# crockwell/far

Hardware: AMD Instinct MI355X
Metric: image-pairs/sec (match+solve+regress) at 640x480 (higher is better)
Workload: dtype f32

## Files before the change

### far_amd/csrc/mlp_fused_f16s.hip

```cpp
#include "common.h"

namespace {

typedef _Float16 f16x8 __attribute__((ext_vector_type(8)));
typedef __attribute__((address_space(3))) void* lptr_t;

constexpr int DM = 128;
constexpr int KIN = 2 * DM;
constexpr int HID = 2 * DM;
constexpr int NS1 = KIN / 16;
constexpr int HT = HID / 32;
constexpr int CT = DM / 32;
constexpr int SLAB = 16384;
constexpr int NSLAB = NS1 + HT;
constexpr int RING = 3;
constexpr int WAVES = 4;
constexpr int PIECES = 16 / WAVES;
constexpr float ACT_SCALE = 16.0f;

__device__ __forceinline__ void glds16(const void* gsrc, unsigned lds_dst_uniform) {
    unsigned keep;
    asm volatile("s_mov_b32 %0, m0\n\ts_mov_b32 m0, %2\n\ts_nop 0\n\tglobal_load_lds_dwordx4 %1, off\n\ts_mov_b32 m0, %0"
                 : "=&s"(keep) : "v"(gsrc), "s"(lds_dst_uniform) : "memory");
}

__device__ __forceinline__ void split8(const float4& u, const float4& v, float scale, f16x8& hi, f16x8& lo) {
    const float x[8] = {u.x, u.y, u.z, u.w, v.x, v.y, v.z, v.w};
#pragma unroll
    for (int i = 0; i < 8; i += 2) {
        f16x2 h, l;
        split2(f32x2{x[i], x[i + 1]} * f32x2{scale, scale}, h, l);
        hi[i] = h.x; hi[i + 1] = h.y;
        lo[i] = l.x; lo[i + 1] = l.y;
    }
}

#define FAR_DPP_F(v, ctrl) __builtin_bit_cast(float, __builtin_amdgcn_update_dpp(0, __builtin_bit_cast(int, v), ctrl, 0xF, 0xF, true))
__device__ __forceinline__ float sum32(float v) {
    v += FAR_DPP_F(v, 0xB1);
    v += FAR_DPP_F(v, 0x4E);
    v += FAR_DPP_F(v, 0x141);
    v += FAR_DPP_F(v, 0x140);
    return v + shfl_xor_f(v, 16);
}


template <bool SPLIT, bool LGKM = true>
__global__ __launch_bounds__(256, 2) void k_mlp128(const float* __restrict__ x, const float* __restrict__ msg,
                                                   const unsigned char* __restrict__ wimg, long R, float hscale, float oscale,
                                                   const float* __restrict__ gamma, const float* __restrict__ beta, float eps,
                                                   float* __restrict__ out, int* __restrict__ overflow) {
    __shared__ __attribute__((aligned(16))) unsigned char ring[RING * SLAB];
    __shared__ __attribute__((aligned(16))) unsigned char xs[WAVES * 4096];
    const int tid = threadIdx.x, lane = tid & 63, l31 = lane & 31, h = lane >> 5;
    const int wave = __builtin_amdgcn_readfirstlane(tid >> 6);
    const long row0 = (long)blockIdx.x * (32 * WAVES) + 32 * wave;
    const unsigned ring_base = (unsigned)__builtin_amdgcn_readfirstlane((int)(unsigned)(size_t)(lptr_t)ring);
    const unsigned xs_base = (unsigned)__builtin_amdgcn_readfirstlane((int)(unsigned)(size_t)(lptr_t)(xs + wave * 4096));
    const unsigned char* wsrc = wimg + (size_t)lane * 16;
    auto request_w = [&](int s) {
        const unsigned dst = ring_base + (unsigned)((s % RING) * SLAB);
#pragma unroll
        for (int i = 0; i < PIECES; ++i)
            glds16(wsrc + (size_t)s * SLAB + (wave + WAVES * i) * 1024, dst + (wave + WAVES * i) * 1024);
    };
    const int rr = lane >> 3, q = lane & 7;
    auto request_x = [&](int c) {
        const float* base = (c < 4 ? x : msg) + 32 * (c & 3);
        const unsigned dst = xs_base;
#pragma unroll
        for (int j = 0; j < 4; ++j) {
            const int r = 8 * j + rr;
            long gr = row0 + r;
            gr = gr < R ? gr : R - 1;
            glds16(base + gr * DM + 4 * (q ^ ((r ^ (r >> 3)) & 7)), dst + j * 1024);
        }
    };
    request_x(0);
    request_w(0);
    request_w(1);
    f16x8 xh[2], xl[2];
    f32x16 acc1[HT];
#pragma unroll
    for (int t = 0; t < HT; ++t)
#pragma unroll
        for (int r = 0; r < 16; ++r) acc1[t][r] = 0.f;
    const unsigned char* xrd = xs + wave * 4096 + (l31 >> 3) * 1024 + (l31 & 7) * 128;
    const int sw = (l31 ^ (l31 >> 3)) & 7;

#pragma unroll
    for (int s = 0; s < NS1; ++s) {
        asm volatile("s_waitcnt vmcnt(0)" ::: "memory");
        ring_barrier<LGKM>();
        if ((s & 1) == 0) {
            float4 raw[4];
#pragma unroll
            for (int i = 0; i < 4; ++i) raw[i] = *reinterpret_cast<const float4*>(xrd + (((4 * h + i) ^ sw) * 16));
            asm volatile("s_waitcnt lgkmcnt(0)" ::: "memory");
            if ((s >> 1) + 1 < KIN / 32) request_x((s >> 1) + 1);
            split8(raw[0], raw[1], ACT_SCALE, xh[0], xl[0]);
            split8(raw[2], raw[3], ACT_SCALE, xh[1], xl[1]);
        }
        request_w(s + 2);
        const unsigned char* slab = ring + (s % RING) * SLAB + lane * 16;
        const f16x8 bh = xh[s & 1], bl = xl[s & 1];
        f16x8 ah[3], al[3];
#pragma unroll
        for (int t = 0; t < 2; ++t) {
            ah[t] = *reinterpret_cast<const f16x8*>(slab + t * 2048);
            al[t] = *reinterpret_cast<const f16x8*>(slab + t * 2048 + 1024);
        }
#pragma unroll
        for (int t = 0; t < HT; ++t) {
            if (t + 2 < HT) {
                ah[(t + 2) % 3] = *reinterpret_cast<const f16x8*>(slab + (t + 2) * 2048);
                al[(t + 2) % 3] = *reinterpret_cast<const f16x8*>(slab + (t + 2) * 2048 + 1024);
            }
            acc1[t] = __builtin_amdgcn_mfma_f32_32x32x16_f16(ah[t % 3], bh, acc1[t], 0, 0, 0);
            if (SPLIT) {
                acc1[t] = __builtin_amdgcn_mfma_f32_32x32x16_f16(ah[t % 3], bl, acc1[t], 0, 0, 0);
                acc1[t] = __builtin_amdgcn_mfma_f32_32x32x16_f16(al[t % 3], bh, acc1[t], 0, 0, 0);
            }
            __builtin_amdgcn_sched_group_barrier(0x100, SPLIT ? 2 : 1, 0);
            __builtin_amdgcn_sched_group_barrier(0x008, SPLIT ? 3 : 1, 0);
        }
    }

    f32x16 acc2[CT];
    float hid_chk = 0.f;
#pragma unroll
    for (int ct = 0; ct < CT; ++ct)
#pragma unroll
        for (int r = 0; r < 16; ++r) acc2[ct][r] = 0.f;
#pragma unroll
    for (int t = 0; t < HT; ++t) {
        const int s = NS1 + t;
        asm volatile("s_waitcnt vmcnt(0)" ::: "memory");
        ring_barrier<LGKM>();
        if (s + 2 < NSLAB) request_w(s + 2);
        const unsigned char* slab = ring + (s % RING) * SLAB + lane * 16;
        f16x8 ha[2], hl[2];
#pragma unroll
        for (int u = 0; u < 2; ++u)
#pragma unroll
            for (int e = 0; e < 8; e += 2) {
                hid_chk += acc1[t][8 * u + e] + acc1[t][8 * u + e + 1];
                const f32x2 hv = __builtin_elementwise_max(f32x2{acc1[t][8 * u + e], acc1[t][8 * u + e + 1]} * f32x2{hscale, hscale}, f32x2{0.f, 0.f});
                f16x2 h2, l2;
                split2(hv, h2, l2);
                ha[u][e] = h2.x; ha[u][e + 1] = h2.y;
                hl[u][e] = l2.x; hl[u][e + 1] = l2.y;
            }
        f16x8 bh[3], bl[3];
#pragma unroll
        for (int i = 0; i < 2; ++i) {
            bh[i] = *reinterpret_cast<const f16x8*>(slab + (i * 2) * 1024);
            bl[i] = *reinterpret_cast<const f16x8*>(slab + (i * 2 + 1) * 1024);
        }
#pragma unroll
        for (int i = 0; i < 2 * CT; ++i) {
            if (i + 2 < 2 * CT) {
                bh[(i + 2) % 3] = *reinterpret_cast<const f16x8*>(slab + ((i + 2) * 2) * 1024);
                bl[(i + 2) % 3] = *reinterpret_cast<const f16x8*>(slab + ((i + 2) * 2 + 1) * 1024);
            }
            const int u = i / CT, ct = i % CT;
            acc2[ct] = __builtin_amdgcn_mfma_f32_32x32x16_f16(ha[u], bh[i % 3], acc2[ct], 0, 0, 0);
            if (SPLIT) {
                acc2[ct] = __builtin_amdgcn_mfma_f32_32x32x16_f16(ha[u], bl[i % 3], acc2[ct], 0, 0, 0);
                acc2[ct] = __builtin_amdgcn_mfma_f32_32x32x16_f16(hl[u], bh[i % 3], acc2[ct], 0, 0, 0);
            }
            __builtin_amdgcn_sched_group_barrier(0x100, SPLIT ? 2 : 1, 0);
            __builtin_amdgcn_sched_group_barrier(0x008, SPLIT ? 3 : 1, 0);
        }
    }

    if (overflow) {
        float chk = hid_chk;
#pragma unroll
        for (int ct = 0; ct < CT; ++ct)
#pragma unroll
            for (int r = 0; r < 16; ++r) chk += acc2[ct][r];
        if (__any(!(fabsf(chk) <= FLT_MAX)) && (threadIdx.x & 63) == 0) atomicOr(overflow, 1);
    }
    const float inv_c = 1.0f / (float)DM;
    float g[CT], b[CT];
#pragma unroll
    for (int ct = 0; ct < CT; ++ct) { g[ct] = gamma[32 * ct + l31]; b[ct] = beta[32 * ct + l31]; }
#pragma unroll
    for (int r = 0; r < 16; ++r) {
        float v[CT];
        float sum = 0.f;
#pragma unroll
        for (int ct = 0; ct < CT; ++ct) { v[ct] = acc2[ct][r] * oscale; sum += v[ct]; }
        const float mean = sum32(sum) * inv_c;
        float sq = 0.f;
#pragma unroll
        for (int ct = 0; ct < CT; ++ct) { v[ct] -= mean; sq += v[ct] * v[ct]; }
        const float rstd = 1.0f / sqrtf(sum32(sq) * inv_c + eps);
        const long orow = row0 + mfma32_row(r, h);
        if (orow < R) {
#pragma unroll
            for (int ct = 0; ct < CT; ++ct) {
                const long o = orow * DM + 32 * ct + l31;
                out[o] = x[o] + (v[ct] * rstd * g[ct] + b[ct]);
            }
        }
    }
}

template <bool SPLIT>
int mlp_fused_launch(const float* x, const float* msg, const void* packed, long R, int d_model, float hscale, float oscale,
                     const float* gamma, const float* beta, float eps, float* out, int* overflow, hipStream_t stream) {
    far_clear_errors();
    if (R == 0) return FAR_OK;
    if (!x || !msg || !packed || !gamma || !beta || !out || R < 0 || d_model != DM || out == x || out == msg) return FAR_EINVAL;
    const long nb = (R + 32 * WAVES - 1) / (32 * WAVES);
    if (nb > 0x7fffffffL) return FAR_EINVAL;
#ifdef FAR_RING_EXP
    if (far_get_tuning(11) & 4) {
        hipLaunchKernelGGL((k_mlp128<SPLIT, false>), dim3((unsigned)nb), dim3(64 * WAVES), 0, stream, x, msg, (const unsigned char*)packed, R,
                           hscale, oscale, gamma, beta, eps, out, overflow);
        return far_check_launch();
    }
#endif
    hipLaunchKernelGGL(k_mlp128<SPLIT>, dim3((unsigned)nb), dim3(64 * WAVES), 0, stream, x, msg, (const unsigned char*)packed, R, hscale,
                       oscale, gamma, beta, eps, out, overflow);
    return far_check_launch();
}

}

extern "C" {

size_t far_mlp_fused_packed_bytes(int d_model) { return d_model == DM ? (size_t)NSLAB * SLAB : 0; }

int far_mlp_fused_f16s(const float* x, const float* msg, const void* packed, long R, int d_model, float hscale, float oscale,
                       const float* gamma, const float* beta, float eps, float* out, int* overflow, hipStream_t stream) {
    return mlp_fused_launch<true>(x, msg, packed, R, d_model, hscale, oscale, gamma, beta, eps, out, overflow, stream);
}

int far_mlp_fused_f16(const float* x, const float* msg, const void* packed, long R, int d_model, float hscale, float oscale,
                      const float* gamma, const float* beta, float eps, float* out, int* overflow, hipStream_t stream) {
    return mlp_fused_launch<false>(x, msg, packed, R, d_model, hscale, oscale, gamma, beta, eps, out, overflow, stream);
}

}
```

### far_amd/flags.py

```python
import os
from collections import namedtuple

Switch = namedtuple('Switch', 'env module attr off_value neutral scope doc')
SWITCHES = [
    Switch('FAR_NO_WINO', 'far_amd.ops', 'USE_WINO', False, 'parity', 'inference',
           'stride-1 3x3 convolutions on K9 (direct implicit GEMM) instead of K17 (Winograd F(2x2,3x3)); same operator, other summation'),
    Switch('FAR_NO_PAD', 'far_amd.loftr.backbone', 'PAD_CHANNELS', False, 'bitwise', 'inference',
           'the 196-channel backbone maps stored with 196 channels instead of 208 (zero weights for the extra ones: exact zeros)'),
    Switch('FAR_NO_PREFETCH', 'far_amd.loftr.model:LoFTR', 'head_prefetch', False, 'bitwise', 'inference',
           "the head's feature stage computed inside forward_rt_prediction instead of enqueued behind K1"),
    Switch('FAR_NO_SIDE_STREAM', 'far_amd.loftr.model:LoFTR', 'head_side_stream', False, 'bitwise', 'inference',
           "the head's feature stage on the step's own stream behind K1 (rounds 2-5) instead of on a second stream next to K1 and the fine level"),
    Switch('FAR_FPN_STREAM', 'far_amd.loftr.model:LoFTR', 'fpn_side_stream', True, 'bitwise', 'inference',
           "OPT-IN (1 switches it ON; default off): the FPN's fine branch on a side stream next to the coarse transformer and K1 (-0.6 ms per 32 "
           "pairs; off by default because the roofline launch -- K17 208 -> 208 @ 240x320 -- then shares the GPU and its in-step duration "
           "in a kernel trace is no longer its own)"),
    Switch('FAR_NO_GATHER_FUSE', 'far_amd.loftr.stages:FinePreprocess', 'fused_gather', False, 'bitwise', 'inference',
           'FinePreprocess.merge_feat on a materialised window tensor (K3 gather + K9) instead of K9 reading through the match indices'),
    Switch('FAR_NO_KV', 'far_amd.loftr.transformer:LoFTREncoderLayer', 'fused_kv', False, 'parity', 'inference',
           "k, v projections + K5's first half as separate launches instead of K9's k|v epilogue (the K'^T V sum changes order)"),
    Switch('FAR_NO_QAPPLY', 'far_amd.loftr.transformer:LoFTREncoderLayer', 'fused_apply', False, 'parity', 'inference',
           "q projection + K5's second half as separate launches instead of K9's attention-apply epilogue (q no longer stays in split operands)"),
    Switch('FAR_NO_STACK', 'far_amd.loftr.transformer:LocalFeatureTransformer', 'stack_self', False, 'bitwise', 'inference',
           "the two 'self' calls of an encoder layer on the two images separately instead of one call on both"),
    Switch('FAR_NO_BN', 'far_amd.ops', 'USE_HIP_BATCHNORM_TRAIN', False, 'parity', 'training',
           'training-mode BatchNorm on nn.BatchNorm2d + torch activations instead of K19 (tests/test_train_kernels_gpu.py holds K19 to the module)'),
]

ENV_ONLY = {
    'FAR_HIP_LIB': ('load', 'path of another build of libfar_hip.so (tools/ab_build.py: same-box A/B against a git revision); skips the build-id check'),
    'FAR_TUNING': ('load', 'comma-separated key=value pairs handed to far_set_tuning at load time, e.g. FAR_TUNING="10=1,8=1" (keys below)'),
    'FAR_SKIP_ASM_CHECK': ('build', "1: far_amd/build.py does not scan the generated code (K9's asm pixel loads; the LDS-DMA ring rule of every kernel with global_load_lds; the half-register writes of the asm fp16 split) after recompiling"),
    'FAR_EXTRA_HIPCC_FLAGS': ('build', 'extra hipcc flags of an experiment build (-DFAR_WINO_EXP=..., tools/wino_exp.sh); part of the build id'),
    'FAR_COMMIT': ('tools', 'commit stamp tools/collect_profiles.sh / tools/step_floors.py write into the profile files'),
    'FAR_C3_PY_NODE': ('bench', "bench.py --workload c3: the encoder layer's autograd node driven from Python instead of far_enc_layer_fwd / _bwd"),
    'FAR_C3_NO_OVERLAP': ('bench', 'bench.py --workload c3: the layer node without side streams'),
    'FAR_C3_PER_OP': ('bench', 'bench.py --workload c3: one autograd node per operator instead of per layer'),
    'FAR_TORCH_ADAMW': ('bench', 'bench.py --workload c3: torch.optim.AdamW instead of K20'),
    'FAR_CUDNN_BENCHMARK': ('bench', 'bench.py: torch.backends.cudnn.benchmark for the vendor comparison legs'),
}

Tuning = namedtuple('Tuning', 'key default values neutral doc')
TUNING = [
    Tuning(0, 3, (0, 1, 2, 4, 7), 'bitwise', 'bit mask of exact-f32 kernels that stagger wave-slot priorities: 1 k_stats, 2 k_match, 4 k_emm_pv'),
    Tuning(1, 0, (1,), 'parity', 'K1 exact-f32 variant: the other tile shape (another summation order of the row statistics)'),
    Tuning(2, 0, (1,), 'bitwise', 'conf_matrix writer variant A (store pattern)'),
    Tuning(3, 0, (1,), 'bitwise', 'conf_matrix writer variant B (store pattern)'),
    Tuning(4, 0, (1,), 'bitwise', 'K9 without the seven-tile mode / K5 windows on the generic path'),
    Tuning(5, 0, (1, 2, 4), 'bitwise', 'K5 apply: tiles per unit'),
    Tuning(6, 0, (64, 256), 'parity', "K5: tokens per K'^T V chunk (another partial-sum grouping)"),
    Tuning(7, 0, (1,), 'bitwise', 'K9 Linear launches always on full-height tiles'),
    Tuning(8, 0, (1,), 'bitwise', 'K17 splits its operands with the five-instruction split2 instead of v_fma_mix (same values)'),
    Tuning(9, 0, (1,), 'bitwise', 'K17 runs a short last channel block on the full body'),
    Tuning(10, 0, (1,), 'bitwise', "K1's match pass without the tile prescreen"),
    Tuning(11, 0, (1, 2), 'bitwise', "K14's pipeline: 0 = 4 waves / 3 slots / counted waits, two workgroups per CU; 1 = 8 waves / 4 slots / counted, one per CU (round 5's form); 2 = 4 waves / 3 slots / vmcnt(0) per phase (fallback without a wait table)"),
    Tuning(12, 0, (1,), 'parity', "K10's inference form on the exact-f32 matrix instruction instead of split fp16"),
    Tuning(15, 0, (1,), 'bitwise', 'K17: 1 = the multiplying wave group does NOT raise its issue priority (the round-4 kernel)'),
    Tuning(13, 0, (1,), 'bitwise', "K9's FPN-merge epilogue in its generic form everywhere"),
]


def off(env):
    if env not in {s.env for s in SWITCHES}:
        raise KeyError(f'{env} is not a registered far_amd switch (far_amd/flags.py)')
    return os.environ.get(env, '0') not in ('', '0')


def value(env, default=None):
    if env not in ENV_ONLY:
        raise KeyError(f'{env} is not a registered far_amd environment variable (far_amd/flags.py)')
    return os.environ.get(env, default)


def known():
    return {s.env for s in SWITCHES} | set(ENV_ONLY)


def unknown_in_environment():
    skip = ('FAR_WINO_', 'FAR_K9_')
    return sorted(k for k in os.environ if k.startswith('FAR_') and k not in known() and not k.startswith(skip))


def target(sw):
    import importlib
    mod, _, cls = sw.module.partition(':')
    obj = importlib.import_module(mod)
    return (getattr(obj, cls) if cls else obj), sw.attr
```

Before: 371.7.

## Double-buffer MLP input chunks, count vmcnt waits, batch residual loads

The fused MLP kernel gets a second per-wave LDS input slot so each activation chunk is requested two phases ahead. The blanket vmcnt(0) waits are replaced by counted waits taken from a compile-time table, so a phase waits only for the loads it actually reads. The epilogue also fetches all residual x values in one batch before the layer norm, and uses an unguarded store path for full tiles. LDS moves to dynamic shared memory, which raises per-block usage by one more input buffer per wave and could reduce occupancy. A tuning knob keeps the older variants available.

```diff
diff --git a/far_amd/csrc/mlp_fused_f16s.hip b/far_amd/csrc/mlp_fused_f16s.hip
--- a/far_amd/csrc/mlp_fused_f16s.hip
+++ b/far_amd/csrc/mlp_fused_f16s.hip
@@ -1,4 +1,5 @@
 #include "common.h"
+#include <type_traits>
 
 namespace {
 
@@ -16,6 +17,7 @@
 constexpr int RING = 3;
 constexpr int WAVES = 4;
 constexpr int PIECES = 16 / WAVES;
+constexpr int XBUF = 4096;
 constexpr float ACT_SCALE = 16.0f;
 
 __device__ __forceinline__ void glds16(const void* gsrc, unsigned lds_dst_uniform) {
@@ -44,19 +46,59 @@
     return v + shfl_xor_f(v, 16);
 }
 
-
-template <bool SPLIT, bool LGKM = true>
+constexpr int chunk_read_in_phase(int s) { return (s < NS1 && (s & 1) == 0) ? s / 2 : -1; }
+constexpr int vm_allow(int p, int xb) {
+    int kind[64] = {}, id[64] = {}, n[64] = {}, cnt = 0;
+    for (int c0 = 0; c0 < xb; ++c0) { kind[cnt] = 0; id[cnt] = c0; n[cnt++] = 4; }
+    for (int s0 = 0; s0 < RING - 1; ++s0) { kind[cnt] = 1; id[cnt] = s0; n[cnt++] = PIECES; }
+    for (int s = 0; s < p; ++s) {
+        const int c = chunk_read_in_phase(s);
+        if (c >= 0 && c + xb < KIN / 32) { kind[cnt] = 0; id[cnt] = c + xb; n[cnt++] = 4; }
+        if (s + RING - 1 < NSLAB) { kind[cnt] = 1; id[cnt] = s + RING - 1; n[cnt++] = PIECES; }
+    }
+    const int cx = chunk_read_in_phase(p);
+    int last = -1;
+    for (int i = 0; i < cnt; ++i)
+        if ((kind[i] == 1 && id[i] == p) || (kind[i] == 0 && id[i] == cx)) last = i;
+    int after = 0;
+    for (int i = last + 1; i < cnt; ++i) after += n[i];
+    return after;
+}
+struct VmTable {
+    int a[NSLAB];
+    constexpr VmTable(int xb) : a{} {
+        for (int p = 0; p < NSLAB; ++p) a[p] = vm_allow(p, xb);
+    }
+};
+static_assert(vm_allow(0, 2) == 4 && vm_allow(1, 2) == 8 && vm_allow(2, 2) == 4 && vm_allow(11, 2) == 8 && vm_allow(12, 2) == 4 && vm_allow(13, 2) == 4 &&
+              vm_allow(15, 2) == 4 && vm_allow(16, 2) == 4 && vm_allow(22, 2) == 4 && vm_allow(23, 2) == 0, "the two-slot / counted schedule");
+static_assert(vm_allow(0, 1) == 4 && vm_allow(1, 1) == 8 && vm_allow(2, 1) == 4 && vm_allow(13, 1) == 8 && vm_allow(14, 1) == 4 && vm_allow(15, 1) == 4 &&
+              vm_allow(23, 1) == 0, "the one-slot / counted schedule");
+
+__device__ __forceinline__ void wait_vm(int n) {
+#define FAR_VM_CASE(k) case k: asm volatile("s_waitcnt vmcnt(" #k ")" ::: "memory"); break;
+    switch (n) {
+        FAR_VM_CASE(0) FAR_VM_CASE(1) FAR_VM_CASE(2) FAR_VM_CASE(3) FAR_VM_CASE(4) FAR_VM_CASE(5) FAR_VM_CASE(6) FAR_VM_CASE(7) FAR_VM_CASE(8)
+        default: asm volatile("s_waitcnt vmcnt(0)" ::: "memory"); break;
+    }
+#undef FAR_VM_CASE
+}
+
+
+template <bool SPLIT, int XB, bool CNT, bool RES, bool LGKM = true>
 __global__ __launch_bounds__(256, 2) void k_mlp128(const float* __restrict__ x, const float* __restrict__ msg,
                                                    const unsigned char* __restrict__ wimg, long R, float hscale, float oscale,
                                                    const float* __restrict__ gamma, const float* __restrict__ beta, float eps,
                                                    float* __restrict__ out, int* __restrict__ overflow) {
-    __shared__ __attribute__((aligned(16))) unsigned char ring[RING * SLAB];
-    __shared__ __attribute__((aligned(16))) unsigned char xs[WAVES * 4096];
+    constexpr VmTable vmt(XB);
+    extern __shared__ __attribute__((aligned(16))) unsigned char smem[];
+    unsigned char* const ring = smem;
+    unsigned char* const xs = smem + RING * SLAB;
     const int tid = threadIdx.x, lane = tid & 63, l31 = lane & 31, h = lane >> 5;
     const int wave = __builtin_amdgcn_readfirstlane(tid >> 6);
     const long row0 = (long)blockIdx.x * (32 * WAVES) + 32 * wave;
     const unsigned ring_base = (unsigned)__builtin_amdgcn_readfirstlane((int)(unsigned)(size_t)(lptr_t)ring);
-    const unsigned xs_base = (unsigned)__builtin_amdgcn_readfirstlane((int)(unsigned)(size_t)(lptr_t)(xs + wave * 4096));
+    const unsigned xs_base = (unsigned)__builtin_amdgcn_readfirstlane((int)(unsigned)(size_t)(lptr_t)(xs + wave * (XB * XBUF)));
     const unsigned char* wsrc = wimg + (size_t)lane * 16;
     auto request_w = [&](int s) {
         const unsigned dst = ring_base + (unsigned)((s % RING) * SLAB);
@@ -67,7 +109,7 @@
     const int rr = lane >> 3, q = lane & 7;
     auto request_x = [&](int c) {
         const float* base = (c < 4 ? x : msg) + 32 * (c & 3);
-        const unsigned dst = xs_base;
+        const unsigned dst = xs_base + (c % XB) * XBUF;
 #pragma unroll
         for (int j = 0; j < 4; ++j) {
             const int r = 8 * j + rr;
@@ -77,6 +119,7 @@
         }
     };
     request_x(0);
+    if (XB == 2) request_x(1);
     request_w(0);
     request_w(1);
     f16x8 xh[2], xl[2];
@@ -85,19 +128,20 @@
     for (int t = 0; t < HT; ++t)
 #pragma unroll
         for (int r = 0; r < 16; ++r) acc1[t][r] = 0.f;
-    const unsigned char* xrd = xs + wave * 4096 + (l31 >> 3) * 1024 + (l31 & 7) * 128;
+    const unsigned char* xrd = xs + wave * (XB * XBUF) + (l31 >> 3) * 1024 + (l31 & 7) * 128;
     const int sw = (l31 ^ (l31 >> 3)) & 7;
 
 #pragma unroll
     for (int s = 0; s < NS1; ++s) {
-        asm volatile("s_waitcnt vmcnt(0)" ::: "memory");
+        wait_vm(CNT ? vmt.a[s] : 0);
         ring_barrier<LGKM>();
         if ((s & 1) == 0) {
+            const int c = s >> 1;
             float4 raw[4];
 #pragma unroll
-            for (int i = 0; i < 4; ++i) raw[i] = *reinterpret_cast<const float4*>(xrd + (((4 * h + i) ^ sw) * 16));
+            for (int i = 0; i < 4; ++i) raw[i] = *reinterpret_cast<const float4*>(xrd + (c % XB) * XBUF + (((4 * h + i) ^ sw) * 16));
             asm volatile("s_waitcnt lgkmcnt(0)" ::: "memory");
-            if ((s >> 1) + 1 < KIN / 32) request_x((s >> 1) + 1);
+            if (c + XB < KIN / 32) request_x(c + XB);
             split8(raw[0], raw[1], ACT_SCALE, xh[0], xl[0]);
             split8(raw[2], raw[3], ACT_SCALE, xh[1], xl[1]);
         }
@@ -135,7 +179,7 @@
 #pragma unroll
     for (int t = 0; t < HT; ++t) {
         const int s = NS1 + t;
-        asm volatile("s_waitcnt vmcnt(0)" ::: "memory");
+        wait_vm(CNT ? vmt.a[s] : 0);
         ring_barrier<LGKM>();
         if (s + 2 < NSLAB) request_w(s + 2);
         const unsigned char* slab = ring + (s % RING) * SLAB + lane * 16;
@@ -182,30 +226,45 @@
             for (int r = 0; r < 16; ++r) chk += acc2[ct][r];
         if (__any(!(fabsf(chk) <= FLT_MAX)) && (threadIdx.x & 63) == 0) atomicOr(overflow, 1);
     }
+    float xres[16][CT];
+    if (RES) {
+#pragma unroll
+        for (int r = 0; r < 16; ++r) {
+            long orow = row0 + mfma32_row(r, h);
+            orow = orow < R ? orow : R - 1;
+#pragma unroll
+            for (int ct = 0; ct < CT; ++ct) xres[r][ct] = x[orow * DM + 32 * ct + l31];
+        }
+    }
     const float inv_c = 1.0f / (float)DM;
     float g[CT], b[CT];
 #pragma unroll
     for (int ct = 0; ct < CT; ++ct) { g[ct] = gamma[32 * ct + l31]; b[ct] = beta[32 * ct + l31]; }
-#pragma unroll
-    for (int r = 0; r < 16; ++r) {
-        float v[CT];
-        float sum = 0.f;
-#pragma unroll
-        for (int ct = 0; ct < CT; ++ct) { v[ct] = acc2[ct][r] * oscale; sum += v[ct]; }
-        const float mean = sum32(sum) * inv_c;
-        float sq = 0.f;
-#pragma unroll
-        for (int ct = 0; ct < CT; ++ct) { v[ct] -= mean; sq += v[ct] * v[ct]; }
-        const float rstd = 1.0f / sqrtf(sum32(sq) * inv_c + eps);
-        const long orow = row0 + mfma32_row(r, h);
-        if (orow < R) {
-#pragma unroll
-            for (int ct = 0; ct < CT; ++ct) {
-                const long o = orow * DM + 32 * ct + l31;
-                out[o] = x[o] + (v[ct] * rstd * g[ct] + b[ct]);
-            }
-        }
-    }
+    auto ln_store = [&](auto all_rows) {
+        constexpr bool ALL = decltype(all_rows)::value;
+#pragma unroll
+        for (int r = 0; r < 16; ++r) {
+            float v[CT];
+            float sum = 0.f;
+#pragma unroll
+            for (int ct = 0; ct < CT; ++ct) { v[ct] = acc2[ct][r] * oscale; sum += v[ct]; }
+            const float mean = sum32(sum) * inv_c;
+            float sq = 0.f;
+#pragma unroll
+            for (int ct = 0; ct < CT; ++ct) { v[ct] -= mean; sq += v[ct] * v[ct]; }
+            const float rstd = 1.0f / sqrtf(sum32(sq) * inv_c + eps);
+            const long orow = row0 + mfma32_row(r, h);
+            if (ALL || orow < R) {
+#pragma unroll
+                for (int ct = 0; ct < CT; ++ct) {
+                    const long o = orow * DM + 32 * ct + l31;
+                    out[o] = (RES ? xres[r][ct] : x[o]) + (v[ct] * rstd * g[ct] + b[ct]);
+                }
+            }
+        }
+    };
+    if (RES && row0 + 32 <= R) ln_store(std::true_type{});
+    else ln_store(std::false_type{});
 }
 
 template <bool SPLIT>
@@ -216,16 +275,25 @@
     if (!x || !msg || !packed || !gamma || !beta || !out || R < 0 || d_model != DM || out == x || out == msg) return FAR_EINVAL;
     const long nb = (R + 32 * WAVES - 1) / (32 * WAVES);
     if (nb > 0x7fffffffL) return FAR_EINVAL;
+    auto launch = [&](auto kern, int smem) -> int {
+        bool cfg_failed = false;
+        FAR_ONCE_PER_DEVICE(cfg_failed = hipFuncSetAttribute((const void*)kern, hipFuncAttributeMaxDynamicSharedMemorySize, smem) != hipSuccess);
+        if (cfg_failed) return far_check_launch();
+        hipLaunchKernelGGL(kern, dim3((unsigned)nb), dim3(64 * WAVES), smem, stream, x, msg, (const unsigned char*)packed, R, hscale, oscale,
+                           gamma, beta, eps, out, overflow);
+        return far_check_launch();
+    };
+    constexpr int SMEM1 = RING * SLAB + WAVES * XBUF, SMEM2 = RING * SLAB + WAVES * 2 * XBUF;
 #ifdef FAR_RING_EXP
-    if (far_get_tuning(11) & 4) {
-        hipLaunchKernelGGL((k_mlp128<SPLIT, false>), dim3((unsigned)nb), dim3(64 * WAVES), 0, stream, x, msg, (const unsigned char*)packed, R,
-                           hscale, oscale, gamma, beta, eps, out, overflow);
-        return far_check_launch();
-    }
+    if (far_get_tuning(11) & 4)
+        return launch(k_mlp128<SPLIT, 1, false, false, false>, SMEM1);
 #endif
-    hipLaunchKernelGGL(k_mlp128<SPLIT>, dim3((unsigned)nb), dim3(64 * WAVES), 0, stream, x, msg, (const unsigned char*)packed, R, hscale,
-                       oscale, gamma, beta, eps, out, overflow);
-    return far_check_launch();
+    switch (far_get_tuning(14)) {
+        case 1: return launch(k_mlp128<SPLIT, 1, false, false>, SMEM1);
+        case 2: return launch(k_mlp128<SPLIT, 1, true, false>, SMEM1);
+        case 3: return launch(k_mlp128<SPLIT, 2, true, false>, SMEM2);
+        default: return launch(k_mlp128<SPLIT, 2, true, true>, SMEM2);
+    }
 }
 
 }
diff --git a/far_amd/flags.py b/far_amd/flags.py
--- a/far_amd/flags.py
+++ b/far_amd/flags.py
@@ -57,6 +57,7 @@
     Tuning(12, 0, (1,), 'parity', "K10's inference form on the exact-f32 matrix instruction instead of split fp16"),
     Tuning(15, 0, (1,), 'bitwise', 'K17: 1 = the multiplying wave group does NOT raise its issue priority (the round-4 kernel)'),
     Tuning(13, 0, (1,), 'bitwise', "K9's FPN-merge epilogue in its generic form everywhere"),
+    Tuning(14, 0, (1, 2, 3), 'bitwise', "K13's input pipeline: 0 = two input slots per wave / counted waits / residual requested in one batch; 1 = one slot, vmcnt(0) per phase, residual row by row (the form before it); 2 = one slot, counted waits; 3 = two slots, counted waits, residual row by row"),
 ]
 
 
```

After: 372.1 (median of 3 runs). About the same (+0.1%).
